# ArseneAmoya/image-retrieval-wavelet

Hardware: AMD Instinct MI355X
Metric: query images/sec + mAP@5000, MIRFLICKR-25k 64-bit hash, 1/2/4/8 MI355X (higher is better)
Workload: dtype f32; 1 GPU; c1: MIRFLICKR-25k shape, retrieval-only: per GPU per step 2048 query images 3x224x224 u8 -> SWT db2 L3 -> band-attention head (Nq=4, E=384; DINOv2 backbone out of scope, CLS features synthetic) -> 64-bit hash -> Hamming top-5000 vs 25,000 codes -> mAP@5000; queries_per_gpu=2048, db_codes=25000, nbits=64, k=5000, wavelet=db2, level=3, arithmetic=fp32 SWT and head (fp32 MFMA), 64-bit popcount ranking, AP in fp32/fp64, streams=1, clock_steps=40, backend=none, parallelism=single GPU

## Files before the change

### image-retrieval-wavelet_amd/csrc/common.hpp

```cpp
#pragma once
#include <hip/hip_runtime.h>
#include <hip/hip_bf16.h>
#include <algorithm>
#include <cstdlib>
#include <cstdio>
#include <cstring>
#include <stdint.h>
#include <stdio.h>
#include <stdarg.h>

#include "twin.hpp"

namespace wv {

const char *tune(const char *name);

#define WV_CHECK_LAUNCH(what)                                                        \
    do {                                                                             \
        hipError_t e_ = hipGetLastError();                                           \
        if (e_ != hipSuccess) WV_FAIL(WV_EHIP, "%s: %s", what, hipGetErrorString(e_)); \
    } while (0)

static inline int64_t ceil_div(int64_t a, int64_t b) { return (a + b - 1) / b; }
static inline int64_t align_up(int64_t a, int64_t b) { return ceil_div(a, b) * b; }

size_t dist_prepared_bytes(int64_t N, int words);
int dist_prepare(const uint64_t *db, void *dbP, int64_t N, int words, hipStream_t st);

constexpr int kWave = 64;
constexpr int kMaxLdsBytes = 160 * 1024;

__device__ __forceinline__ int lane_id() { return threadIdx.x & 63; }
__device__ __forceinline__ int wave_id() { return threadIdx.x >> 6; }

__device__ __forceinline__ uint32_t own_byte(int v)
{
    asm volatile("" : "+v"(v));
    return (uint32_t)v;
}

__device__ __forceinline__ int mbcnt(uint64_t mask)
{
    return __builtin_amdgcn_mbcnt_hi((uint32_t)(mask >> 32),
                                     __builtin_amdgcn_mbcnt_lo((uint32_t)mask, 0));
}

__device__ __forceinline__ uint32_t wave_incl_scan_u32(uint32_t v)
{
    v += (uint32_t)__builtin_amdgcn_update_dpp(0, (int)v, 0x111, 0xf, 0xf, false);
    v += (uint32_t)__builtin_amdgcn_update_dpp(0, (int)v, 0x112, 0xf, 0xf, false);
    v += (uint32_t)__builtin_amdgcn_update_dpp(0, (int)v, 0x114, 0xf, 0xf, false);
    v += (uint32_t)__builtin_amdgcn_update_dpp(0, (int)v, 0x118, 0xf, 0xf, false);
    v += (uint32_t)__builtin_amdgcn_update_dpp(0, (int)v, 0x142, 0xa, 0xf, false);
    v += (uint32_t)__builtin_amdgcn_update_dpp(0, (int)v, 0x143, 0xc, 0xf, false);
    return v;
}

__device__ __forceinline__ uint32_t wave_sum_u32(uint32_t v)
{
    return (uint32_t)__builtin_amdgcn_readlane((int)wave_incl_scan_u32(v), 63);
}

__device__ __forceinline__ double wave_sum_f64(double v)
{
#pragma unroll
    for (int d = 32; d > 0; d >>= 1) v += __shfl_xor(v, d, 64);
    return v;
}

__device__ __forceinline__ float gelu_erf(float v)
{
#ifdef WV_HF_EXACT_ERF
    return 0.5f * v * (1.0f + erff(v * 0.70710678118654752440f));
#else
    const float x = fabsf(v) * 0.70710678118654752440f;
    const float t = __builtin_amdgcn_rcpf(fmaf(0.3275911f, x, 1.0f));
    float p = fmaf(1.061405429f, t, -1.453152027f);
    p = fmaf(p, t, 1.421413741f);
    p = fmaf(p, t, -0.284496736f);
    p = fmaf(p, t, 0.254829592f);
    const float erfc_abs = p * t * __expf(-x * x);
    return 0.5f * v * (v >= 0.f ? 2.0f - erfc_abs : erfc_abs);
#endif
}

}
```

### image-retrieval-wavelet_amd/csrc/head.hip

```cpp
#include "head.hpp"

namespace wv {

template <int TM, int TN, int EPI>
__global__ __launch_bounds__(256) void k_gemm_nt(const float *__restrict__ A, const float *__restrict__ W,
                                                 const float *__restrict__ bias,
                                                 const float *__restrict__ R, int rmod,
                                                 float *__restrict__ C, int M, int N, int K)
{
    const int lane = lane_id(), wv = wave_id();
    const int r = lane & 31, h = lane >> 5;
    const int64_t i0 = (int64_t)blockIdx.y * (64 * TM) + (wv >> 1) * (32 * TM);
    const int64_t j0 = (int64_t)blockIdx.x * (64 * TN) + (wv & 1) * (32 * TN);
    if (i0 >= M || j0 >= N) return;
    f32x16 acc[TM][TN];
#pragma unroll
    for (int a = 0; a < TM; ++a)
#pragma unroll
        for (int b = 0; b < TN; ++b)
#pragma unroll
            for (int e = 0; e < 16; ++e) acc[a][b][e] = 0.f;
    const float *arow[TM], *brow[TN];
#pragma unroll
    for (int a = 0; a < TM; ++a) arow[a] = A + min(i0 + a * 32 + r, (int64_t)M - 1) * K;
// ... 143 lines not shown
            const int lin = blockIdx.y * gridDim.x + blockIdx.x;
            const int tile = (lin % 8) * (total / 8) + lin / 8;
            by = tile / gridDim.x;
            bx = tile - by * gridDim.x;
        }
    }
    const int64_t m0 = (int64_t)by * BM, n0 = (int64_t)bx * BN;

    f32x16 acc[3];
#pragma unroll
    for (int b = 0; b < 3; ++b)
#pragma unroll
        for (int e = 0; e < 16; ++e) acc[b][e] = 0.f;

    f32x4 ra[A4], rb[B4];
    const float *ga[A4], *gb[B4];
    int so_a[A4], so_b[B4];
#pragma unroll
    for (int i = 0; i < A4; ++i) {
        const int ch = i * 256 + tid, row = ch / CPR, c4 = ch % CPR;
        ga[i] = A + min(m0 + row, (int64_t)M - 1) * K + 4 * c4;
        so_a[i] = row * LDP + 4 * c4;
    }
#pragma unroll
    for (int i = 0; i < B4; ++i) {
        const int ch = i * 256 + tid, row = ch / CPR, c4 = ch % CPR;
        gb[i] = W + min(n0 + row, (int64_t)N - 1) * K + 4 * c4;
        so_b[i] = BM * LDP + row * LDP + 4 * c4;
    }
    constexpr int STAGE = (BM + BN) * LDP;
#pragma unroll
    for (int i = 0; i < A4; ++i) ra[i] = *reinterpret_cast<const f32x4 *>(ga[i]);
#pragma unroll
    for (int i = 0; i < B4; ++i) rb[i] = *reinterpret_cast<const f32x4 *>(gb[i]);
#pragma unroll
    for (int i = 0; i < A4; ++i) *reinterpret_cast<f32x4 *>(sm + so_a[i]) = ra[i];
#pragma unroll
    for (int i = 0; i < B4; ++i) *reinterpret_cast<f32x4 *>(sm + so_b[i]) = rb[i];
    const int nk = kchunk / BK;
    if (nk > 1) {
#pragma unroll
        for (int i = 0; i < A4; ++i) ra[i] = *reinterpret_cast<const f32x4 *>(ga[i] + BK);
#pragma unroll
        for (int i = 0; i < B4; ++i) rb[i] = *reinterpret_cast<const f32x4 *>(gb[i] + BK);
    }
    __syncthreads();
    for (int kt = 0; kt < nk; ++kt) {
        float *cur = sm + (kt & 1) * STAGE;
        float *nxt = sm + ((kt & 1) ^ 1) * STAGE;
        if (kt + 1 < nk) {
#pragma unroll
            for (int i = 0; i < A4; ++i) *reinterpret_cast<f32x4 *>(nxt + so_a[i]) = ra[i];
#pragma unroll
            for (int i = 0; i < B4; ++i) *reinterpret_cast<f32x4 *>(nxt + so_b[i]) = rb[i];
        }
        if (kt + 2 < nk) {
            const int k0 = (kt + 2) * BK;
#pragma unroll
            for (int i = 0; i < A4; ++i) ra[i] = *reinterpret_cast<const f32x4 *>(ga[i] + k0);
#pragma unroll
            for (int i = 0; i < B4; ++i) rb[i] = *reinterpret_cast<const f32x4 *>(gb[i] + k0);
        }
        const float *as = cur + (wv * 32 + r) * LDP + 4 * h;
        const float *bs = cur + BM * LDP + r * LDP + 4 * h;
        f32x4 av_n = *reinterpret_cast<const f32x4 *>(as), bv_n[3];
#pragma unroll
        for (int b = 0; b < 3; ++b) bv_n[b] = *reinterpret_cast<const f32x4 *>(bs + b * 32 * LDP);
#pragma unroll
        for (int c = 0; c < BK / 8; ++c) {
            const f32x4 av = av_n;
            f32x4 bv[3];
#pragma unroll
            for (int b = 0; b < 3; ++b) bv[b] = bv_n[b];
            if (c + 1 < BK / 8) {
                av_n = *reinterpret_cast<const f32x4 *>(as + 8 * (c + 1));
#pragma unroll
                for (int b = 0; b < 3; ++b) bv_n[b] = *reinterpret_cast<const f32x4 *>(bs + b * 32 * LDP + 8 * (c + 1));
            }
            __builtin_amdgcn_sched_barrier(0);
#pragma unroll
            for (int b = 0; b < 3; ++b) acc[b] = __builtin_amdgcn_mfma_f32_32x32x2f32(av.x, bv[b].x, acc[b], 0, 0, 0);
#pragma unroll
            for (int b = 0; b < 3; ++b) acc[b] = __builtin_amdgcn_mfma_f32_32x32x2f32(av.y, bv[b].y, acc[b], 0, 0, 0);
#pragma unroll
            for (int b = 0; b < 3; ++b) acc[b] = __builtin_amdgcn_mfma_f32_32x32x2f32(av.z, bv[b].z, acc[b], 0, 0, 0);
#pragma unroll
            for (int b = 0; b < 3; ++b) acc[b] = __builtin_amdgcn_mfma_f32_32x32x2f32(av.w, bv[b].w, acc[b], 0, 0, 0);
        }
        __syncthreads();
    }
    const int64_t row0 = m0 + wv * 32 + 4 * h, col0 = n0 + r;
    if (m0 + BM <= M && n0 + BN <= N) {
#pragma unroll
        for (int b = 0; b < 3; ++b) store_block<EPI, false, true>(acc[b], row0, col0 + b * 32, bias, R, rmod, C, M, N);
    } else {
#pragma unroll
        for (int b = 0; b < 3; ++b) store_block<EPI, true, true>(acc[b], row0, col0 + b * 32, bias, R, rmod, C, M, N);
    }
}

__global__ __launch_bounds__(256) void k_attn_core(const float *__restrict__ Qp,
                                                   const float *__restrict__ KV,
                                                   float *__restrict__ ctx, int B, int E, int heads,
                                                   int Nq, int S)
{
    extern __shared__ float4 sm4[];
    float *kv = reinterpret_cast<float *>(sm4);
    const int KP = 2 * E + 4;
    float *q = kv + (size_t)S * KP;
    float *P = q + (size_t)Nq * E;
    const int b = blockIdx.x, tid = threadIdx.x;
    const int hd = E / heads;
    const float scale = 1.0f / sqrtf((float)hd);
    const int row4 = 2 * E / 4;
    for (int t = tid; t < S * row4; t += blockDim.x) {
        const int s = t / row4, c = t - s * row4;
        *reinterpret_cast<float4 *>(kv + (size_t)s * KP + 4 * c) =
            *reinterpret_cast<const float4 *>(KV + ((size_t)s * B + b) * 2 * E + 4 * c);
    }
    for (int t = tid; t < Nq * E / 4; t += blockDim.x)
        *reinterpret_cast<float4 *>(q + 4 * t) = *reinterpret_cast<const float4 *>(Qp + 4 * t);
    __syncthreads();
    const int ndots = Nq * heads * S;
    for (int t = tid; t < ndots; t += blockDim.x) {
        const int s = t % S, hh = (t / S) % heads, i = t / (S * heads);
        const float *qv = q + (size_t)i * E + hh * hd;
        const float *kr = kv + (size_t)s * KP + hh * hd;
        float acc = 0.f;
        for (int d = 0; d < hd; ++d) acc = fmaf(qv[d], kr[d], acc);
        P[t] = acc * scale;
    }
    __syncthreads();
    for (int t = tid; t < Nq * heads; t += blockDim.x) {
        float *p = P + (size_t)t * S;
        float mx = p[0];
        for (int s = 1; s < S; ++s) mx = fmaxf(mx, p[s]);
        float sum = 0.f;
        for (int s = 0; s < S; ++s) {
            p[s] = expf(p[s] - mx);
            sum += p[s];
        }
        for (int s = 0; s < S; ++s) p[s] = p[s] / sum;
    }
    __syncthreads();
    for (int t = tid; t < Nq * E; t += blockDim.x) {
        const int e = t % E, i = t / E, hh = e / hd;
        const float *p = P + ((size_t)i * heads + hh) * S;
        float acc = 0.f;
        for (int s = 0; s < S; ++s) acc = fmaf(p[s], kv[(size_t)s * KP + E + e], acc);
        ctx[((size_t)b * Nq + i) * E + e] = acc;
    }
}

template <int NV>
__global__ __launch_bounds__(256) void k_layernorm(const float *__restrict__ x, const float *__restrict__ w,
                                                   const float *__restrict__ bvec, float *__restrict__ y,
                                                   int64_t rows, int E, float eps, int nparts)
{
    const int lane = lane_id();
    const int64_t row = (int64_t)blockIdx.x * 4 + wave_id();
    if (row >= rows) return;
    const float *xr = x + row * E;
    const size_t pstride = (size_t)rows * E;
    auto value = [&](int e) {
        float a = xr[e];
        for (int q = 1; q < nparts; ++q) a += xr[q * pstride + e];
        return a;
    };
    float val[NV > 0 ? NV : 1];
    float s = 0.f;
    if constexpr (NV > 0) {
#pragma unroll
        for (int j = 0; j < NV; ++j) {
            const int e = lane + 64 * j;
            val[j] = e < E ? value(e) : 0.f;
            s += val[j];
        }
    } else {
        for (int e = lane; e < E; e += 64) s += value(e);
    }
#pragma unroll
    for (int d = 32; d > 0; d >>= 1) s += __shfl_xor(s, d, 64);
    const float mean = s / (float)E;
    float v = 0.f;
    if constexpr (NV > 0) {
#pragma unroll
        for (int j = 0; j < NV; ++j) {
            const float dlt = lane + 64 * j < E ? val[j] - mean : 0.f;
            v = fmaf(dlt, dlt, v);
        }
    } else {
        for (int e = lane; e < E; e += 64) {
            const float dlt = value(e) - mean;
            v = fmaf(dlt, dlt, v);
        }
    }
#pragma unroll
    for (int d = 32; d > 0; d >>= 1) v += __shfl_xor(v, d, 64);
    const float rstd = 1.0f / sqrtf(v / (float)E + eps);
    if constexpr (NV > 0) {
#pragma unroll
        for (int j = 0; j < NV; ++j) {
            const int e = lane + 64 * j;
            if (e < E) y[row * E + e] = (val[j] - mean) * rstd * w[e] + bvec[e];
        }
    } else {
        for (int e = lane; e < E; e += 64) y[row * E + e] = (value(e) - mean) * rstd * w[e] + bvec[e];
    }
}

void launch_layernorm(const float *x, const float *w, const float *b, float *y, int64_t rows, int E, float eps, int nparts,
                      hipStream_t st)
{
    const dim3 grid((unsigned)ceil_div(rows, 4));
    if (E <= 512) hipLaunchKernelGGL(k_layernorm<8>, grid, dim3(256), 0, st, x, w, b, y, rows, E, eps, nparts);
    else if (E <= 1024) hipLaunchKernelGGL(k_layernorm<16>, grid, dim3(256), 0, st, x, w, b, y, rows, E, eps, nparts);
    else hipLaunchKernelGGL(k_layernorm<0>, grid, dim3(256), 0, st, x, w, b, y, rows, E, eps, nparts);
}

__global__ __launch_bounds__(256) void k_qproj(const float *__restrict__ q, const float *__restrict__ W,
                                               const float *__restrict__ b, float *__restrict__ Qp, int Nq, int E)
{
    const int lane = lane_id(), o = blockIdx.x * 4 + wave_id();
    if (o >= Nq * E) return;
    const int n = o / E, e = o - n * E;
    const float *wr = W + (size_t)e * E, *qr = q + (size_t)n * E;
    float a = 0.f;
    for (int k = lane; k < E; k += 64) a = fmaf(qr[k], wr[k], a);
#pragma unroll
    for (int d = 32; d > 0; d >>= 1) a += __shfl_xor(a, d, 64);
    if (lane == 0) Qp[o] = a + b[e];
}

__global__ void k_mean_rows(const float *__restrict__ x, float *__restrict__ y, int64_t groups, int n, int E)
{
    const int64_t total = groups * E;
    for (int64_t i = (int64_t)blockIdx.x * blockDim.x + threadIdx.x; i < total;
         i += (int64_t)gridDim.x * blockDim.x) {
        const int64_t g = i / E;
        const int e = (int)(i - g * E);
        float s = 0.f;
        for (int j = 0; j < n; ++j) s += x[(g * n + j) * E + e];
        y[i] = s / (float)n;
    }
}

__global__ __launch_bounds__(256) void k_hash_tail(const float *__restrict__ fused, int B, int E,
                                                   const float *__restrict__ hw, const float *__restrict__ hb,
                                                   const float *__restrict__ bn_w, const float *__restrict__ bn_b,
                                                   const float *__restrict__ bn_mean,
                                                   const float *__restrict__ bn_var, float eps, int nbits,
                                                   float *__restrict__ logits_out,
                                                   float *__restrict__ codes_out,
                                                   uint64_t *__restrict__ packed_out)
{
    extern __shared__ float xrow[];
    const int b = blockIdx.x, tid = threadIdx.x, lane = lane_id();
    for (int e = tid; e < E; e += blockDim.x) xrow[e] = fused[(size_t)b * E + e];
    __syncthreads();
    const int words = (nbits + 63) / 64;
    for (int j0 = 0; j0 < words * 64; j0 += blockDim.x) {
        const int j = j0 + tid;
        float v = 0.f;
        const bool valid = j < nbits;
        if (valid) {
            const float4 *wr = reinterpret_cast<const float4 *>(hw + (size_t)j * E);
            float acc = 0.f;
            for (int e4 = 0; e4 < E / 4; ++e4) {
                const float4 w4 = wr[e4];
                acc = fmaf(w4.x, xrow[4 * e4 + 0], acc);
                acc = fmaf(w4.y, xrow[4 * e4 + 1], acc);
                acc = fmaf(w4.z, xrow[4 * e4 + 2], acc);
                acc = fmaf(w4.w, xrow[4 * e4 + 3], acc);
            }
            v = acc + (hb ? hb[j] : 0.f);
            if (bn_w) v = (v - bn_mean[j]) / sqrtf(bn_var[j] + eps) * bn_w[j] + bn_b[j];
            if (logits_out) logits_out[(size_t)b * nbits + j] = v;
            if (codes_out) codes_out[(size_t)b * nbits + j] = v > 0.f ? 1.f : (v < 0.f ? -1.f : (v == 0.f ? 0.f : v));
        }
        const uint64_t word = __ballot(valid && v > 0.f);
        if (packed_out && lane == 0 && j < words * 64) packed_out[(size_t)b * words + j / 64] = word;
    }
}

__global__ __launch_bounds__(256) void k_hash_tail16(const float *__restrict__ fused, int B, int E,
                                                     const float *__restrict__ hw, const float *__restrict__ hb,
                                                     const float *__restrict__ bn_w, const float *__restrict__ bn_b,
                                                     const float *__restrict__ bn_mean,
                                                     const float *__restrict__ bn_var, float eps, int nbits,
                                                     float *__restrict__ logits_out,
                                                     float *__restrict__ codes_out,
                                                     uint64_t *__restrict__ packed_out)
{
    extern __shared__ float4 hsm4[];
    float4 *xs4 = hsm4;
    float *Wt = reinterpret_cast<float *>(hsm4 + 4 * E);
    const int tid = threadIdx.x, lane = lane_id(), wv = wave_id();
    const int b0 = blockIdx.x * 16;
    {
        float *xs = reinterpret_cast<float *>(xs4);
#pragma unroll 8
        for (int i = tid; i < 16 * E; i += 256) {
            const int sidx = i / E, e = i - sidx * E, b = b0 + sidx;
            xs[((sidx >> 2) * E + e) * 4 + (sidx & 3)] = b < B ? fused[(size_t)b * E + e] : 0.f;
        }
    }
    const int words = (nbits + 63) / 64, E4 = E / 4;
    for (int wd = 0; wd < words; ++wd) {
        __syncthreads();
        constexpr int UN = 8;
        for (int base = 0; base < 64 * E4; base += 256 * UN) {
            f32x4 w4[UN];
#pragma unroll
            for (int u = 0; u < UN; ++u) {
                const int i = base + u * 256 + tid, jj = i / E4, e4 = i - jj * E4, j = wd * 64 + jj;
                w4[u] = f32x4{0.f, 0.f, 0.f, 0.f};
                if (i < 64 * E4 && j < nbits) w4[u] = *reinterpret_cast<const f32x4 *>(hw + (size_t)j * E + 4 * e4);
            }
#pragma unroll
            for (int u = 0; u < UN; ++u) {
                const int i = base + u * 256 + tid, jj = i / E4, e4 = i - jj * E4;
                if (i < 64 * E4) {
                    Wt[(4 * e4 + 0) * 65 + jj] = w4[u].x;
                    Wt[(4 * e4 + 1) * 65 + jj] = w4[u].y;
                    Wt[(4 * e4 + 2) * 65 + jj] = w4[u].z;
                    Wt[(4 * e4 + 3) * 65 + jj] = w4[u].w;
                }
            }
        }
        __syncthreads();
        const int j = wd * 64 + lane;
        const bool valid = j < nbits;
        float a0 = 0.f, a1 = 0.f, a2 = 0.f, a3 = 0.f;
        const float4 *xw = xs4 + wv * E;
#pragma unroll 16
        for (int e = 0; e < E; ++e) {
            const float w = Wt[e * 65 + lane];
            const float4 x = xw[e];
            a0 = fmaf(w, x.x, a0);
            a1 = fmaf(w, x.y, a1);
            a2 = fmaf(w, x.z, a2);
            a3 = fmaf(w, x.w, a3);
        }
        float scale = 1.f, shift = 0.f, mean = 0.f, bias = 0.f;
        if (valid) {
            bias = hb ? hb[j] : 0.f;
            if (bn_w) { mean = bn_mean[j]; scale = sqrtf(bn_var[j] + eps); shift = bn_b[j]; }
        }
        const float acc[4] = {a0, a1, a2, a3};
#pragma unroll
        for (int u = 0; u < 4; ++u) {
            const int b = b0 + 4 * wv + u;
            float v = acc[u] + bias;
            if (bn_w && valid) v = (v - mean) / scale * bn_w[j] + shift;
            const bool on = valid && b < B;
            if (on) {
                if (logits_out) logits_out[(size_t)b * nbits + j] = v;
                if (codes_out) codes_out[(size_t)b * nbits + j] = v > 0.f ? 1.f : (v < 0.f ? -1.f : (v == 0.f ? 0.f : v));
            }
            const uint64_t word = __ballot(on && v > 0.f);
            if (packed_out && lane == 0 && b < B) packed_out[(size_t)b * words + wd] = word;
        }
    }
}

__global__ __launch_bounds__(256) void k_hash_tail_mfma(const float *__restrict__ fused, int B, int E,
                                                        const float *__restrict__ hw, const float *__restrict__ hb,
                                                        const float *__restrict__ bn_w, const float *__restrict__ bn_b,
                                                        const float *__restrict__ bn_mean,
                                                        const float *__restrict__ bn_var, float eps, int nbits,
                                                        float *__restrict__ logits_out, float *__restrict__ codes_out,
                                                        uint64_t *__restrict__ packed_out)
{
    __shared__ float part[4][16][64];
    const int lane = lane_id(), wv = wave_id(), r = lane & 31, h = lane >> 5;
    const int b0 = blockIdx.x * 32, n = blockIdx.y;
    const int cpw = E / 32;
    const float *arow = fused + (size_t)min(b0 + r, B - 1) * E + (size_t)wv * cpw * 8 + 4 * h;
    const float *brow = hw + (size_t)min(n * 32 + r, nbits - 1) * E + (size_t)wv * cpw * 8 + 4 * h;
    f32x16 acc[2];
#pragma unroll
    for (int i = 0; i < 2; ++i)
#pragma unroll
        for (int e = 0; e < 16; ++e) acc[i][e] = 0.f;
    constexpr int CB = 12;
    for (int c0 = 0; c0 < cpw; c0 += CB) {
        f32x4 av[CB], bv[CB];
#pragma unroll
        for (int u = 0; u < CB; ++u) {
            const int c = min(c0 + u, cpw - 1);
            av[u] = *reinterpret_cast<const f32x4 *>(arow + 8 * c);
            bv[u] = *reinterpret_cast<const f32x4 *>(brow + 8 * c);
        }
#pragma unroll
        for (int u = 0; u < CB; ++u) {
            if (c0 + u < cpw) {
                acc[u & 1] = __builtin_amdgcn_mfma_f32_32x32x2f32(av[u].x, bv[u].x, acc[u & 1], 0, 0, 0);
                acc[u & 1] = __builtin_amdgcn_mfma_f32_32x32x2f32(av[u].y, bv[u].y, acc[u & 1], 0, 0, 0);
                acc[u & 1] = __builtin_amdgcn_mfma_f32_32x32x2f32(av[u].z, bv[u].z, acc[u & 1], 0, 0, 0);
                acc[u & 1] = __builtin_amdgcn_mfma_f32_32x32x2f32(av[u].w, bv[u].w, acc[u & 1], 0, 0, 0);
            }
        }
    }
#pragma unroll
    for (int e = 0; e < 16; ++e) part[wv][e][lane] = acc[0][e] + acc[1][e];
    __syncthreads();
    const int words = (nbits + 63) / 64;
    const int j = 32 * n + r;
    const bool valid = j < nbits;
    float bias = 0.f, mean = 0.f, scale = 1.f, gain = 1.f, shift = 0.f;
    if (valid) {
        bias = hb ? hb[j] : 0.f;
        if (bn_w) { mean = bn_mean[j]; scale = sqrtf(bn_var[j] + eps); gain = bn_w[j]; shift = bn_b[j]; }
    }
#pragma unroll
    for (int ee = 0; ee < 4; ++ee) {
        const int e = 4 * wv + ee;
        const int b = b0 + 8 * (e >> 2) + 4 * h + (e & 3);
        float v = ((part[0][e][lane] + part[1][e][lane]) + part[2][e][lane]) + part[3][e][lane];
        v += bias;
        if (bn_w) v = (v - mean) / scale * gain + shift;
        if (valid && b < B) {
            if (logits_out) logits_out[(size_t)b * nbits + j] = v;
            if (codes_out) codes_out[(size_t)b * nbits + j] = v > 0.f ? 1.f : (v < 0.f ? -1.f : (v == 0.f ? 0.f : v));
        }
        const uint64_t bal = __ballot(valid && v > 0.f);
        if (packed_out && r == 0 && b < B)
            reinterpret_cast<uint32_t *>(packed_out)[((size_t)b * words + (n >> 1)) * 2 + (n & 1)] = (uint32_t)(bal >> (32 * h));
    }
    if (packed_out && n == (int)gridDim.y - 1 && (gridDim.y & 1) && wv == 0 && lane < 32 && b0 + lane < B)
        reinterpret_cast<uint32_t *>(packed_out)[((size_t)(b0 + lane) * words + (n >> 1)) * 2 + 1] = 0u;
}

template <int TM, int TN, int EPI>
static void launch_gemm_nt(const float *A, const float *W, const float *bias, const float *R, int rmod, float *C,
                           int M, int N, int K, hipStream_t st)
{
    dim3 grid((unsigned)ceil_div(N, 64 * TN), (unsigned)ceil_div(M, 64 * TM));
    hipLaunchKernelGGL((k_gemm_nt<TM, TN, EPI>), grid, dim3(256), 0, st, A, W, bias, R, rmod, C, M, N, K);
}

template <int BM, int BN, int EPI>
static void launch_gemm_lds(const float *A, const float *W, const float *bias, const float *R, int rmod, float *C,
                            int M, int N, int K, hipStream_t st)
{
    constexpr size_t lds = (size_t)2 * (BM + BN) * 36 * sizeof(float);
    auto kern = k_gemm_lds<BM, BN, EPI>;
    if (lds > 64 * 1024)
        (void)hipFuncSetAttribute(reinterpret_cast<const void *>(kern), hipFuncAttributeMaxDynamicSharedMemorySize, (int)lds);
    dim3 grid((unsigned)ceil_div(N, BN), (unsigned)ceil_div(M, BM));
    hipLaunchKernelGGL(kern, grid, dim3(256), lds, st, A, W, bias, R, rmod, C, M, N, K);
}

template <int BK, int EPI>
static void launch_gemm_panel(const float *A, const float *W, const float *bias, const float *R, int rmod, float *C,
                              int M, int N, int K, int ksplit, hipStream_t st)
{
    constexpr size_t lds = (size_t)2 * (128 + 96) * (BK + 4) * sizeof(float);
    auto kern = k_gemm_panel<BK, EPI>;
    if (lds > 64 * 1024)
        (void)hipFuncSetAttribute(reinterpret_cast<const void *>(kern), hipFuncAttributeMaxDynamicSharedMemorySize, (int)lds);
    dim3 grid((unsigned)ceil_div(N, 96), (unsigned)ceil_div(M, 128), (unsigned)ksplit);
    hipLaunchKernelGGL(kern, grid, dim3(256), lds, st, A, W, bias, R, rmod, C, M, N, K, K / ksplit);
}

struct PathF32 {
    using Hidden = float;
    template <int EPI>
    static void gemm(GemmPlan g, const float *A, const float *W, const float *bias, const float *R, int rmod, float *C, int M,
                     int N, int K, hipStream_t st)
    {
        switch (g.kernel) {
        case Gemm::nt64: return launch_gemm_nt<1, 1, EPI>(A, W, bias, R, rmod, C, M, N, K, st);
        case Gemm::nt128: return launch_gemm_nt<2, 2, EPI>(A, W, bias, R, rmod, C, M, N, K, st);
        case Gemm::lds64: return launch_gemm_lds<64, 64, EPI>(A, W, bias, R, rmod, C, M, N, K, st);
        case Gemm::lds128x64: return launch_gemm_lds<128, 64, EPI>(A, W, bias, R, rmod, C, M, N, K, st);
        case Gemm::lds128: return launch_gemm_lds<128, 128, EPI>(A, W, bias, R, rmod, C, M, N, K, st);
        case Gemm::panel32: return launch_gemm_panel<32, EPI>(A, W, bias, R, rmod, C, M, N, K, g.ksplit, st);
        case Gemm::panel64: return launch_gemm_panel<64, EPI>(A, W, bias, R, rmod, C, M, N, K, g.ksplit, st);
        default: return;
        }
    }
};

void launch_gemm_f32(GemmPlan g, const float *A, const float *W, const float *bias, float *C, int M, int N, int K, hipStream_t st)
{
    PathF32::gemm<EPI_NONE>(g, A, W, bias, nullptr, 1, C, M, N, K, st);
}

void launch_qproj(const wv_head_params *p, float *Qp, hipStream_t st)
{
    hipLaunchKernelGGL(k_qproj, dim3((unsigned)ceil_div(p->num_queries * p->embed_dim, 4)), dim3(256), 0, st, p->q_eff,
                       p->in_proj_w, p->in_proj_b, Qp, p->num_queries, p->embed_dim);
}

void launch_attn_core(const wv_head_params *p, const HeadPlan &pl, const float *Qp, const float *KV, float *ctx, int B, hipStream_t st)
{
    if (pl.attn_lds > 64 * 1024)
        (void)hipFuncSetAttribute(reinterpret_cast<const void *>(k_attn_core), hipFuncAttributeMaxDynamicSharedMemorySize,
                                  (int)pl.attn_lds);
    hipLaunchKernelGGL(k_attn_core, dim3(B), dim3(256), pl.attn_lds, st, Qp, KV, ctx, B, p->embed_dim, p->num_heads,
                       p->num_queries, p->num_tokens);
}

void launch_mean_rows(const float *x, float *y, int64_t groups, int n, int E, hipStream_t st)
{
    hipLaunchKernelGGL(k_mean_rows, dim3((unsigned)std::min<int64_t>(ceil_div(groups * E, 256), 4096)), dim3(256), 0, st, x, y,
                       groups, n, E);
}

}

using namespace wv;

extern "C" size_t wv_band_attn_pool_workspace_bytes(const wv_head_params *p, int B)
{
    return head_plan(p, B, HeadPrec::f32).ws.bytes;
}

extern "C" int wv_band_attn_qproj(const wv_head_params *p, float *q_proj_out, void *stream)
{
    HeadPlan pl{};
    if (!head_check_params(p, 1, pl)) WV_FAIL(pl.rc, "%s", pl.why);
    WV_REQUIRE(q_proj_out, "band_attn_qproj: null buffer");
    launch_qproj(p, q_proj_out, (hipStream_t)stream);
    WV_CHECK_LAUNCH("k_qproj");
    return WV_OK;
}

extern "C" size_t wv_band_attn_prepared_bytes(const wv_head_params *p)
{
    if (!p) return 0;
    const HeadPlan pl = head_plan(p, 1, HeadPrec::f32);
    if (pl.rc) {
        set_error("%s", pl.why);
        return 0;
    }
    return head_front_prepared_bytes(p);
}

extern "C" int wv_band_attn_prepare(const wv_head_params *p, void *prepared_out, void *stream)
{
    HeadPlan pl{};
    if (!head_check_params(p, 1, pl)) WV_FAIL(pl.rc, "%s", pl.why);
    WV_REQUIRE(prepared_out, "band_attn_prepare: null buffer");
    if (!head_front_has_kernel(p))
        WV_FAIL(WV_ENOTSUP, "band_attn_prepare: no fused kernel for E=%d S=%d Nq=%d heads=%d", p->embed_dim, p->num_tokens,
                p->num_queries, p->num_heads);
    return head_front_prepare(p, prepared_out, (hipStream_t)stream);
}

extern "C" int wv_band_attn_pool(const wv_head_params *p, const float *feats, int B, float *out,
                                 void *workspace, size_t workspace_bytes, void *stream)
{
    const HeadPlan pl = head_plan(p, B, HeadPrec::f32);
    if (pl.rc) WV_FAIL(pl.rc, "%s", pl.why);
    WV_REQUIRE(feats && out, "band_attn_pool: null buffer");
    WV_REQUIRE((int64_t)B * std::max(p->num_queries, p->num_tokens) < (1ll << 31), "band_attn_pool: B=%d too large", B);
    if (B == 0) return WV_OK;
    if (!workspace || workspace_bytes < pl.ws.bytes)
        WV_FAIL(WV_ENOMEM, "band_attn_pool: workspace %zu < %zu bytes", workspace_bytes, pl.ws.bytes);
    hipStream_t st = (hipStream_t)stream;
    const float *Qp = p->q_proj ? p->q_proj : reinterpret_cast<const float *>(p->prepared);
    if (!Qp && !pl.front) {
        launch_qproj(p, ws_at<float>(workspace, pl.ws.Qp), st);
        Qp = ws_at<float>(workspace, pl.ws.Qp);
    }
    const size_t E = p->embed_dim;
    const HeadWeights<float> w{p->in_proj_w + E * E, p->attn_out_w, p->mlp0_w, p->mlp2_w, p->out_w};
    head_run_stages<PathF32>(p, pl, w, Qp, feats, B, out, workspace, st);
    WV_CHECK_LAUNCH("band_attn_pool");
    return WV_OK;
}

extern "C" int wv_hash_tail(const float *fused, int B, int E, const float *hash_w, const float *hash_b,
                            const float *bn_w, const float *bn_b, const float *bn_mean,
                            const float *bn_var, float bn_eps, int nbits, float *logits_out,
                            float *codes_out, uint64_t *packed_out, void *stream)
{
    WV_REQUIRE(fused && hash_w, "hash_tail: null buffer");
    WV_REQUIRE(B >= 0 && E >= 4 && E % 4 == 0 && nbits >= 1, "hash_tail: bad shape B=%d E=%d nbits=%d", B, E, nbits);
    WV_REQUIRE(!bn_w || (bn_b && bn_mean && bn_var), "hash_tail: incomplete BatchNorm parameters");
    WV_REQUIRE(E * sizeof(float) <= 48 * 1024, "hash_tail: E=%d too large", E);
    if (B == 0) return WV_OK;
    const size_t lds16 = ((size_t)4 * E * 4 + (size_t)E * 65) * sizeof(float);
    const char *pin = ::wv::tune("WV_HASH_TAIL");
    const bool simple = pin && !strcmp(pin, "simple");
    if (!simple && !(pin && !strcmp(pin, "valu16")) && E % 32 == 0 && (B >= 32 || (pin && !strcmp(pin, "mfma")))) {
        const dim3 grid((unsigned)ceil_div(B, 32), (unsigned)ceil_div(nbits, 32));
        hipLaunchKernelGGL(k_hash_tail_mfma, grid, dim3(256), 0, (hipStream_t)stream, fused, B, E, hash_w, hash_b, bn_w, bn_b,
                           bn_mean, bn_var, bn_eps, nbits, logits_out, codes_out, packed_out);
    } else if (lds16 <= (size_t)kMaxLdsBytes - 1024 && B >= 64 && !simple) {
        if (lds16 > 64 * 1024)
            (void)hipFuncSetAttribute(reinterpret_cast<const void *>(k_hash_tail16), hipFuncAttributeMaxDynamicSharedMemorySize, (int)lds16);
        hipLaunchKernelGGL(k_hash_tail16, dim3((unsigned)ceil_div(B, 16)), dim3(256), lds16, (hipStream_t)stream, fused, B,
                           E, hash_w, hash_b, bn_w, bn_b, bn_mean, bn_var, bn_eps, nbits, logits_out, codes_out,
                           packed_out);
    } else {
        hipLaunchKernelGGL(k_hash_tail, dim3(B), dim3(256), E * sizeof(float), (hipStream_t)stream, fused, B, E,
                           hash_w, hash_b, bn_w, bn_b, bn_mean, bn_var, bn_eps, nbits, logits_out, codes_out,
                           packed_out);
    }
    WV_CHECK_LAUNCH("k_hash_tail");
    return WV_OK;
}
```

### image-retrieval-wavelet_amd/csrc/head_front.hip

```cpp
#include "head.hpp"

namespace wv {

constexpr int HF_E = 384;
constexpr int HF_LDA = HF_E + 4;
constexpr int HF_KC = HF_E / 8;
constexpr int HF_D = 4;
constexpr int HF_ENTRY4 = 3 * 64;
constexpr int HF_TILE = 32 * HF_LDA;

struct HeadFrontPlan {
    int ok, nq, heads, nsc, kw, ns;
    int nsp;
    size_t entries;
    size_t wave_stride4;
    size_t qp_bytes, bytes;
};

static HeadFrontPlan head_front_plan(const wv_head_params *p)
{
    HeadFrontPlan g{};
    if (!p || p->embed_dim != HF_E || p->num_tokens != 4 || (p->num_queries != 4 && p->num_queries != 8)) return g;
    if (p->num_heads < 1 || HF_E % p->num_heads) return g;
    const int cols = p->num_queries * p->num_heads;
// ... 46 lines not shown
                a[1] = fmaf(qv[d], kv.y, a[1]);
                a[2] = fmaf(qv[d], kv.z, a[2]);
                a[3] = fmaf(qv[d], kv.w, a[3]);
            }
            v = f32x4{a[0] * scale, a[1] * scale, a[2] * scale, a[3] * scale};
        }
    } else if (entry >= (size_t)nsp && entry < entries) {
        size_t m = entry - nsp;
        const int n = 96 * w + 32 * slot + r;
        const float *src;
        if (m < (size_t)HF_KC) src = in_proj_w + (size_t)2 * E * E + (size_t)n * E + 8 * m + 4 * h;
        else if (m < (size_t)2 * HF_KC) src = Wo + (size_t)n * E + 8 * (m - HF_KC) + 4 * h;
        else {
            m -= 2 * HF_KC;
            const int j = (int)(m / (2 * HF_KC)), mm = (int)(m % (2 * HF_KC));
            if (mm < HF_KC) src = W0 + (size_t)(E * j + n) * E + 8 * mm + 4 * h;
            else src = W2 + (size_t)n * (4 * E) + E * j + 8 * (mm - HF_KC) + 4 * h;
        }
        v = *reinterpret_cast<const f32x4 *>(src);
    }
    stream[idx] = v;
}

#ifdef WV_HF_STAMPS
__device__ unsigned long long g_hf_stamps[16];
#define HF_STAMP(i) do { __builtin_amdgcn_sched_barrier(0); const unsigned long long now_ = __builtin_amdgcn_s_memtime(); \
    asm volatile("s_waitcnt lgkmcnt(0)" ::: "memory"); if (threadIdx.x == 0) atomicAdd(&g_hf_stamps[i], now_ - stamp_); stamp_ = now_; \
    __builtin_amdgcn_sched_barrier(0); } while (0)
#define HF_STAMP_INIT unsigned long long stamp_ = __builtin_amdgcn_s_memtime()
#else
#define HF_STAMP(i) do { } while (0)
#define HF_STAMP_INIT do { } while (0)
#endif

__device__ __forceinline__ void lds_barrier() { asm volatile("s_waitcnt lgkmcnt(0)\n\ts_barrier" ::: "memory"); }

#define HF_MFMA(a, b, c) __builtin_amdgcn_mfma_f32_32x32x2f32((a), (b), (c), 0, 0, 0)


template <int NE>
__device__ __forceinline__ void gemm_stream(f32x16 (&acc)[3], f32x4 (&ring)[HF_D][3], const f32x4 *&wq, const float *arow)
{
    static_assert(NE % HF_D == 0, "phase length must be a multiple of the ring depth");
    f32x4 av_n = *reinterpret_cast<const f32x4 *>(arow);
    for (int c = 0; c < NE; c += HF_D) {
#pragma unroll
        for (int d = 0; d < HF_D; ++d) {
            constexpr int D = HF_D;
            const int slot = (d + D - 1) % D;
            const f32x4 av = av_n;
            const int cn = min(c + d + 1, NE - 1);
            ring[slot][0] = wq[(size_t)(d * 3 + 0) * 64];
            av_n = *reinterpret_cast<const f32x4 *>(arow + 8 * cn);
            __builtin_amdgcn_sched_barrier(0);
#pragma unroll
            for (int b = 0; b < 3; ++b) acc[b] = HF_MFMA(av.x, ring[d][b].x, acc[b]);
            __builtin_amdgcn_sched_barrier(0);
            ring[slot][1] = wq[(size_t)(d * 3 + 1) * 64];
            __builtin_amdgcn_sched_barrier(0);
#pragma unroll
            for (int b = 0; b < 3; ++b) acc[b] = HF_MFMA(av.y, ring[d][b].y, acc[b]);
            __builtin_amdgcn_sched_barrier(0);
            ring[slot][2] = wq[(size_t)(d * 3 + 2) * 64];
            __builtin_amdgcn_sched_barrier(0);
#pragma unroll
            for (int b = 0; b < 3; ++b) acc[b] = HF_MFMA(av.z, ring[d][b].z, acc[b]);
#pragma unroll
            for (int b = 0; b < 3; ++b) acc[b] = HF_MFMA(av.w, ring[d][b].w, acc[b]);
            __builtin_amdgcn_sched_barrier(0);
        }
        wq += (size_t)HF_D * HF_ENTRY4;
    }
}

template <int NE, int NREAL>
__device__ __forceinline__ void scores_stream(f32x16 (&sacc)[3], f32x4 (&ring)[HF_D][3], const f32x4 *&wq, const float *arow)
{
    static_assert(NE % HF_D == 0, "phase length must be a multiple of the ring depth");
    f32x4 a_n[3];
#pragma unroll
    for (int t = 0; t < 3; ++t) a_n[t] = *reinterpret_cast<const f32x4 *>(arow + 8 * t);
    for (int c = 0; c < NE; c += HF_D) {
#pragma unroll
        for (int d = 0; d < HF_D; ++d) {
            constexpr int D = HF_D;
            const int slot = (d + D - 1) % D;
#pragma unroll
            for (int b = 0; b < 3; ++b) ring[slot][b] = wq[(size_t)(d * 3 + b) * 64];
            f32x4 a[3];
#pragma unroll
            for (int t = 0; t < 3; ++t) a[t] = a_n[t];
            const int cn = min(c + d + 1, NREAL - 1);
#pragma unroll
            for (int t = 0; t < 3; ++t) a_n[t] = *reinterpret_cast<const f32x4 *>(arow + 8 * (3 * cn + t));
            __builtin_amdgcn_sched_barrier(0);
#pragma unroll
            for (int t = 0; t < 3; ++t) sacc[t] = HF_MFMA(a[t].x, ring[d][t].x, sacc[t]);
#pragma unroll
            for (int t = 0; t < 3; ++t) sacc[t] = HF_MFMA(a[t].y, ring[d][t].y, sacc[t]);
#pragma unroll
            for (int t = 0; t < 3; ++t) sacc[t] = HF_MFMA(a[t].z, ring[d][t].z, sacc[t]);
#pragma unroll
            for (int t = 0; t < 3; ++t) sacc[t] = HF_MFMA(a[t].w, ring[d][t].w, sacc[t]);
            __builtin_amdgcn_sched_barrier(0);
        }
        wq += (size_t)HF_D * HF_ENTRY4;
    }
}

__device__ __forceinline__ void zero_acc(f32x16 (&acc)[3])
{
#pragma unroll
    for (int b = 0; b < 3; ++b)
#pragma unroll
        for (int e = 0; e < 16; ++e) acc[b][e] = 0.f;
}

__device__ __forceinline__ float half_reduce16(const float (&v)[16], int r)
{
    float a[8], b[4], c[2];
    const bool u4 = r & 16, u3 = r & 8, u2 = r & 4, u1 = r & 2;
#pragma unroll
    for (int k = 0; k < 8; ++k) a[k] = (u4 ? v[k + 8] : v[k]) + __shfl_xor(u4 ? v[k] : v[k + 8], 16, 64);
#pragma unroll
    for (int k = 0; k < 4; ++k) b[k] = (u3 ? a[k + 4] : a[k]) + __shfl_xor(u3 ? a[k] : a[k + 4], 8, 64);
#pragma unroll
    for (int k = 0; k < 2; ++k) c[k] = (u2 ? b[k + 2] : b[k]) + __shfl_xor(u2 ? b[k] : b[k + 2], 4, 64);
    float d = (u1 ? c[1] : c[0]) + __shfl_xor(u1 ? c[0] : c[1], 2, 64);
    d += __shfl_xor(d, 1, 64);
    return d;
}

template <int NQ, int NSC>
__global__ __launch_bounds__(256, 1) void k_head_front(const float *__restrict__ feats, const f32x4 *__restrict__ stream,
                                                       size_t wave_stride4, const float *__restrict__ bv,
                                                       const float *__restrict__ bo, const float *__restrict__ q_eff,
                                                       const float *__restrict__ ln_w, const float *__restrict__ ln_b,
                                                       const float *__restrict__ b0, const float *__restrict__ b2,
                                                       float *__restrict__ x2, int B, int heads, float eps)
{
    constexpr int E = HF_E, LDA = HF_LDA, SPB = 32 / NQ, KW = 4 / NSC, NS = (HF_KC / KW) / 3;
    constexpr int SPP = 33;
    extern __shared__ float4 hf_sm4[];
    float *T0 = reinterpret_cast<float *>(hf_sm4);
    float *H = T0 + HF_TILE;
    float *SP = H;
    float *P = H + 4 * 32 * SPP;
    float *ST = H + HF_TILE;
    const int tid = threadIdx.x, lane = lane_id(), wv = wave_id(), r = lane & 31, h = lane >> 5;
    const int hd = E / heads;
    const int s0 = blockIdx.x * SPB;

    HF_STAMP_INIT;
    f32x4 ring[HF_D][3];
    const f32x4 *wq = stream + (size_t)wv * wave_stride4 + lane;
#pragma unroll
    for (int d = 0; d < HF_D - 1; ++d)
#pragma unroll
        for (int b = 0; b < 3; ++b) ring[d][b] = wq[(size_t)(d * 3 + b) * 64];
    wq += (size_t)(HF_D - 1) * HF_ENTRY4;
    float c_bv[3], c_bo[3], c_lw[3], c_lb[3], c_b2[3], c_b0[4][3], c_q[NQ][3];
#pragma unroll
    for (int b = 0; b < 3; ++b) {
        const int col = 96 * wv + 32 * b + r;
        c_bv[b] = bv[col];
        c_bo[b] = bo[col];
        c_lw[b] = ln_w[col];
        c_lb[b] = ln_b[col];
        c_b2[b] = b2[col];
#pragma unroll
        for (int j = 0; j < 4; ++j) c_b0[j][b] = b0[E * j + col];
#pragma unroll
        for (int i = 0; i < NQ; ++i) c_q[i][b] = q_eff[i * E + col];
    }

    for (int i = tid; i < 32 * (E / 4); i += 256) {
        const int rr = i / (E / 4), c4 = i - rr * (E / 4), bl = rr >> 2, s = rr & 3;
        f32x4 v = {0.f, 0.f, 0.f, 0.f};
        if (bl < SPB && s0 + bl < B) v = *reinterpret_cast<const f32x4 *>(feats + ((size_t)s * B + s0 + bl) * E + 4 * c4);
        *reinterpret_cast<f32x4 *>(T0 + rr * LDA + 4 * c4) = v;
    }
    lds_barrier();
    HF_STAMP(0);
    const float *arow0 = T0 + r * LDA + 4 * h;
    f32x16 acc[3];

    {
        zero_acc(acc);
        const int kpart = wv % KW;
        scores_stream<(NS + HF_D - 1) / HF_D * HF_D, NS>(acc, ring, wq, arow0 + 8 * kpart * (HF_KC / KW));
#pragma unroll
        for (int e = 0; e < 16; ++e) {
            const int row = 8 * (e >> 2) + 4 * h + (e & 3);
            SP[(wv * 32 + row) * SPP + r] = (acc[0][e] + acc[1][e]) + acc[2][e];
        }
    }
    lds_barrier();
    HF_STAMP(1);
    for (int it = tid; it < SPB * NQ * heads; it += 256) {
        const int hh = it % heads, bi = it / heads, bl = bi / NQ, i = bi - bl * NQ;
        const int sc = i * heads + hh, sb = sc >> 5, col = sc & 31;
        float p[4];
#pragma unroll
        for (int s = 0; s < 4; ++s) {
            float a = SP[((sb * KW) * 32 + 4 * bl + s) * SPP + col];
#pragma unroll
            for (int k = 1; k < KW; ++k) a += SP[((sb * KW + k) * 32 + 4 * bl + s) * SPP + col];
            p[s] = a;
        }
        const float mx = fmaxf(fmaxf(p[0], p[1]), fmaxf(p[2], p[3]));
        float sum = 0.f;
#pragma unroll
        for (int s = 0; s < 4; ++s) {
            p[s] = expf(p[s] - mx);
            sum += p[s];
        }
        *reinterpret_cast<f32x4 *>(P + (size_t)it * 4) = f32x4{p[0] / sum, p[1] / sum, p[2] / sum, p[3] / sum};
    }

    HF_STAMP(2);
    zero_acc(acc);
    gemm_stream<HF_KC>(acc, ring, wq, arow0);
    lds_barrier();
    HF_STAMP(3);
#pragma unroll
    for (int b = 0; b < 3; ++b) {
        const int col = 96 * wv + 32 * b + r, hh = col / hd;
        const float bias = c_bv[b];
#pragma unroll
        for (int j = 0; j < 4; ++j) {
            const int bl = h + 2 * j;
            if (bl < SPB) {
                const float v0 = acc[b][4 * j] + bias, v1 = acc[b][4 * j + 1] + bias, v2 = acc[b][4 * j + 2] + bias,
                            v3 = acc[b][4 * j + 3] + bias;
#pragma unroll
                for (int i = 0; i < NQ; ++i) {
                    const f32x4 p4 = *reinterpret_cast<const f32x4 *>(P + ((size_t)(bl * NQ + i) * heads + hh) * 4);
                    float c = p4.x * v0;
                    c = fmaf(p4.y, v1, c);
                    c = fmaf(p4.z, v2, c);
                    c = fmaf(p4.w, v3, c);
                    T0[(bl * NQ + i) * LDA + col] = c;
                }
            }
        }
    }
    lds_barrier();
    HF_STAMP(4);

    zero_acc(acc);
    gemm_stream<HF_KC>(acc, ring, wq, arow0);
    HF_STAMP(5);
    {
        float rs[16];
#pragma unroll
        for (int e = 0; e < 16; ++e) rs[e] = 0.f;
#pragma unroll
        for (int b = 0; b < 3; ++b)
#pragma unroll
            for (int e = 0; e < 16; ++e) {
                const float qv = NQ == 4 ? c_q[e & 3][b] : (h ? c_q[(4 + (e & 3)) % NQ][b] : c_q[e & 3][b]);
                acc[b][e] = acc[b][e] + c_bo[b] + qv;
                rs[e] += acc[b][e];
            }
        const int erow = r >> 1, srow = 8 * (erow >> 2) + 4 * h + (erow & 3);
        {
            const float t = half_reduce16(rs, r);
            if (!(r & 1)) ST[wv * 32 + srow] = t;
        }
        lds_barrier();
        float mean[16];
#pragma unroll
        for (int e = 0; e < 16; ++e) {
            const int row = 8 * (e >> 2) + 4 * h + (e & 3);
            mean[e] = (((ST[row] + ST[32 + row]) + ST[64 + row]) + ST[96 + row]) * (1.0f / (float)E);
            rs[e] = 0.f;
        }
#pragma unroll
        for (int b = 0; b < 3; ++b)
#pragma unroll
            for (int e = 0; e < 16; ++e) {
                acc[b][e] -= mean[e];
                rs[e] = fmaf(acc[b][e], acc[b][e], rs[e]);
            }
        {
            const float t = half_reduce16(rs, r);
            if (!(r & 1)) ST[128 + wv * 32 + srow] = t;
        }
        lds_barrier();
#pragma unroll
        for (int e = 0; e < 16; ++e) {
            const int row = 8 * (e >> 2) + 4 * h + (e & 3);
            const float var = (((ST[128 + row] + ST[160 + row]) + ST[192 + row]) + ST[224 + row]) * (1.0f / (float)E);
            mean[e] = 1.0f / sqrtf(var + eps);
        }
#pragma unroll
        for (int b = 0; b < 3; ++b) {
            const int col = 96 * wv + 32 * b + r;
#pragma unroll
            for (int e = 0; e < 16; ++e) {
                const int row = 8 * (e >> 2) + 4 * h + (e & 3);
                T0[row * LDA + col] = acc[b][e] * mean[e] * c_lw[b] + c_lb[b];
            }
        }
    }
    lds_barrier();
    HF_STAMP(6);

    f32x16 xacc[3];
    zero_acc(xacc);
#pragma unroll 1
    for (int j = 0; j < 4; ++j) {
        zero_acc(acc);
        gemm_stream<HF_KC>(acc, ring, wq, arow0);
        HF_STAMP(7);
        float *Hj = H + (j & 1) * HF_TILE;
#pragma unroll
        for (int b = 0; b < 3; ++b) {
            const int col = 96 * wv + 32 * b + r;
            const float bias = j == 0 ? c_b0[0][b] : j == 1 ? c_b0[1][b] : j == 2 ? c_b0[2][b] : c_b0[3][b];
#pragma unroll
            for (int e = 0; e < 16; ++e) {
                const int row = 8 * (e >> 2) + 4 * h + (e & 3);
                Hj[row * LDA + col] = gelu_erf(acc[b][e] + bias);
            }
        }
        lds_barrier();
        HF_STAMP(8);
        gemm_stream<HF_KC>(xacc, ring, wq, Hj + r * LDA + 4 * h);
        HF_STAMP(9);
    }
#pragma unroll
    for (int b = 0; b < 3; ++b) {
        const int col = 96 * wv + 32 * b + r;
#pragma unroll
        for (int e = 0; e < 16; ++e) {
            const int row = 8 * (e >> 2) + 4 * h + (e & 3);
            const int64_t grow = (int64_t)blockIdx.x * 32 + row;
            if (grow < (int64_t)B * NQ) x2[grow * E + col] = xacc[b][e] + c_b2[b] + T0[row * LDA + col];
        }
    }
    HF_STAMP(10);
}

int head_front_prepare(const wv_head_params *p, void *prepared, hipStream_t st)
{
    const HeadFrontPlan g = head_front_plan(p);
    float *Qp = reinterpret_cast<float *>(prepared);
    launch_qproj(p, Qp, st);
    WV_CHECK_LAUNCH("k_qproj");
    f32x4 *stream = reinterpret_cast<f32x4 *>(reinterpret_cast<char *>(prepared) + g.qp_bytes);
    const size_t total = 4 * g.wave_stride4;
    hipLaunchKernelGGL(k_head_pack, dim3((unsigned)ceil_div((int64_t)total, 256)), dim3(256), 0, st, p->in_proj_w, Qp,
                       p->attn_out_w, p->mlp0_w, p->mlp2_w, stream, g.nq, g.heads, g.kw, g.ns, g.nsp, g.entries, g.wave_stride4);
    WV_CHECK_LAUNCH("k_head_pack");
    return WV_OK;
}

template <int NQ, int NSC>
static void launch_front(const HeadFrontPlan &g, const wv_head_params *p, const float *feats, int B, float *x2, hipStream_t st)
{
    constexpr size_t lds = (size_t)3 * HF_TILE * sizeof(float);
    static_assert(lds <= (size_t)kMaxLdsBytes, "three tiles must fit the CU's LDS");
    auto kern = k_head_front<NQ, NSC>;
    (void)hipFuncSetAttribute(reinterpret_cast<const void *>(kern), hipFuncAttributeMaxDynamicSharedMemorySize, (int)lds);
    const f32x4 *stream = reinterpret_cast<const f32x4 *>(reinterpret_cast<const char *>(p->prepared) + g.qp_bytes);
    hipLaunchKernelGGL(kern, dim3((unsigned)ceil_div(B, 32 / NQ)), dim3(256), lds, st, feats, stream, g.wave_stride4,
                       p->in_proj_b + 2 * HF_E, p->attn_out_b, p->q_eff, p->norm1_w, p->norm1_b, p->mlp0_b, p->mlp2_b, x2, B,
                       p->num_heads, p->ln_eps);
}

void head_front_launch(const wv_head_params *p, const float *feats, int B, float *x2, hipStream_t st)
{
    const HeadFrontPlan g = head_front_plan(p);
    if (g.nq == 4 && g.nsc == 1) launch_front<4, 1>(g, p, feats, B, x2, st);
    else if (g.nq == 4 && g.nsc == 2) launch_front<4, 2>(g, p, feats, B, x2, st);
    else if (g.nq == 4 && g.nsc == 4) launch_front<4, 4>(g, p, feats, B, x2, st);
    else if (g.nq == 8 && g.nsc == 1) launch_front<8, 1>(g, p, feats, B, x2, st);
    else if (g.nq == 8 && g.nsc == 2) launch_front<8, 2>(g, p, feats, B, x2, st);
    else if (g.nq == 8 && g.nsc == 4) launch_front<8, 4>(g, p, feats, B, x2, st);
}

}

#ifdef WV_HF_STAMPS
extern "C" int wv_debug_hf_stamps(unsigned long long *host16)
{
    if (hipMemcpyFromSymbol(host16, HIP_SYMBOL(wv::g_hf_stamps), 16 * sizeof(unsigned long long)) != hipSuccess) return -5;
    unsigned long long zero[16] = {0};
    if (hipMemcpyToSymbol(HIP_SYMBOL(wv::g_hf_stamps), zero, sizeof(zero)) != hipSuccess) return -5;
    return 0;
}
#endif
```

Measured before the change: 1.600 million query images/s.

## Reorder head-front loads, pack GELU in pairs, template layernorm on slice count

The fused head-front kernel now issues the feature-tile global loads into registers first, then the constant loads and the weight-ring prefetch, and only afterwards writes the tile to LDS, with sched barriers to keep that order. The goal is to overlap global load latency. GELU is evaluated two elements at a time with a packed float2 helper, and the residual reads from LDS are hoisted ahead of the output store loop. Layernorm is templated on the number of k-split partial slices and gets an E<=384 instantiation, so partial-sum loads and gain/bias loads are unrolled and issued up front; unsupported slice counts abort. Debug exports are also added. These changes raise register pressure and could lower occupancy.

```diff
diff --git a/image-retrieval-wavelet_amd/csrc/common.hpp b/image-retrieval-wavelet_amd/csrc/common.hpp
--- a/image-retrieval-wavelet_amd/csrc/common.hpp
+++ b/image-retrieval-wavelet_amd/csrc/common.hpp
@@ -84,4 +84,25 @@
 #endif
 }
 
+using f32x2 = __attribute__((ext_vector_type(2))) float;
+__device__ __forceinline__ f32x2 gelu_erf2(f32x2 v)
+{
+#ifdef WV_HF_EXACT_ERF
+    return f32x2{gelu_erf(v.x), gelu_erf(v.y)};
+#else
+    const f32x2 x = __builtin_elementwise_abs(v) * 0.70710678118654752440f;
+    const f32x2 d = __builtin_elementwise_fma(f32x2{0.3275911f, 0.3275911f}, x, f32x2{1.0f, 1.0f});
+    const f32x2 t = {__builtin_amdgcn_rcpf(d.x), __builtin_amdgcn_rcpf(d.y)};
+    f32x2 p = __builtin_elementwise_fma(f32x2{1.061405429f, 1.061405429f}, t, f32x2{-1.453152027f, -1.453152027f});
+    p = __builtin_elementwise_fma(p, t, f32x2{1.421413741f, 1.421413741f});
+    p = __builtin_elementwise_fma(p, t, f32x2{-0.284496736f, -0.284496736f});
+    p = __builtin_elementwise_fma(p, t, f32x2{0.254829592f, 0.254829592f});
+    const f32x2 a = -x * x;
+    const f32x2 erfc_abs = p * t * f32x2{__expf(a.x), __expf(a.y)};
+    const f32x2 two = f32x2{2.0f, 2.0f} - erfc_abs;
+    const f32x2 s = {v.x >= 0.f ? two.x : erfc_abs.x, v.y >= 0.f ? two.y : erfc_abs.y};
+    return 0.5f * v * s;
+#endif
 }
+
+}
diff --git a/image-retrieval-wavelet_amd/csrc/head.hip b/image-retrieval-wavelet_amd/csrc/head.hip
--- a/image-retrieval-wavelet_amd/csrc/head.hip
+++ b/image-retrieval-wavelet_amd/csrc/head.hip
@@ -319,10 +319,10 @@
     }
 }
 
-template <int NV>
+template <int NV, int NP>
 __global__ __launch_bounds__(256) void k_layernorm(const float *__restrict__ x, const float *__restrict__ w,
                                                    const float *__restrict__ bvec, float *__restrict__ y,
-                                                   int64_t rows, int E, float eps, int nparts)
+                                                   int64_t rows, int E, float eps)
 {
     const int lane = lane_id();
     const int64_t row = (int64_t)blockIdx.x * 4 + wave_id();
@@ -330,17 +330,33 @@
     const float *xr = x + row * E;
     const size_t pstride = (size_t)rows * E;
     auto value = [&](int e) {
-        float a = xr[e];
-        for (int q = 1; q < nparts; ++q) a += xr[q * pstride + e];
+        float part[NP];
+#pragma unroll
+        for (int q = 0; q < NP; ++q) part[q] = xr[q * pstride + e];
+        float a = part[0];
+#pragma unroll
+        for (int q = 1; q < NP; ++q) a += part[q];
         return a;
     };
-    float val[NV > 0 ? NV : 1];
+    float val[NV > 0 ? NV : 1], gain[NV > 0 ? NV : 1], shift[NV > 0 ? NV : 1];
     float s = 0.f;
     if constexpr (NV > 0) {
+        float part[NP][NV];
+#pragma unroll
+        for (int q = 0; q < NP; ++q)
+#pragma unroll
+            for (int j = 0; j < NV; ++j) part[q][j] = xr[q * pstride + min(lane + 64 * j, E - 1)];
 #pragma unroll
         for (int j = 0; j < NV; ++j) {
-            const int e = lane + 64 * j;
-            val[j] = e < E ? value(e) : 0.f;
+            gain[j] = w[min(lane + 64 * j, E - 1)];
+            shift[j] = bvec[min(lane + 64 * j, E - 1)];
+        }
+#pragma unroll
+        for (int j = 0; j < NV; ++j) {
+            float a = part[0][j];
+#pragma unroll
+            for (int q = 1; q < NP; ++q) a += part[q][j];
+            val[j] = lane + 64 * j < E ? a : 0.f;
             s += val[j];
         }
     } else {
@@ -369,20 +385,40 @@
 #pragma unroll
         for (int j = 0; j < NV; ++j) {
             const int e = lane + 64 * j;
-            if (e < E) y[row * E + e] = (val[j] - mean) * rstd * w[e] + bvec[e];
+            if (e < E) y[row * E + e] = (val[j] - mean) * rstd * gain[j] + shift[j];
         }
     } else {
         for (int e = lane; e < E; e += 64) y[row * E + e] = (value(e) - mean) * rstd * w[e] + bvec[e];
     }
 }
 
+using LayerNormKernel = void (*)(const float *, const float *, const float *, float *, int64_t, int, float);
+
+template <int NP> static LayerNormKernel layernorm_rows(int E)
+{
+    return E <= 384 ? k_layernorm<6, NP> : E <= 512 ? k_layernorm<8, NP> : E <= 1024 ? k_layernorm<16, NP> : k_layernorm<0, NP>;
+}
+
+static LayerNormKernel layernorm_kernel(int E, int nparts)
+{
+    switch (nparts) {
+    case 1: return layernorm_rows<1>(E);
+    case 2: return layernorm_rows<2>(E);
+    case 4: return layernorm_rows<4>(E);
+    case 8: return layernorm_rows<8>(E);
+    default: return nullptr;
+    }
+}
+
 void launch_layernorm(const float *x, const float *w, const float *b, float *y, int64_t rows, int E, float eps, int nparts,
                       hipStream_t st)
 {
-    const dim3 grid((unsigned)ceil_div(rows, 4));
-    if (E <= 512) hipLaunchKernelGGL(k_layernorm<8>, grid, dim3(256), 0, st, x, w, b, y, rows, E, eps, nparts);
-    else if (E <= 1024) hipLaunchKernelGGL(k_layernorm<16>, grid, dim3(256), 0, st, x, w, b, y, rows, E, eps, nparts);
-    else hipLaunchKernelGGL(k_layernorm<0>, grid, dim3(256), 0, st, x, w, b, y, rows, E, eps, nparts);
+    const LayerNormKernel kern = layernorm_kernel(E, nparts);
+    if (!kern) {
+        fprintf(stderr, "wvhash: k_layernorm has no instantiation for %d slices\n", nparts);
+        abort();
+    }
+    hipLaunchKernelGGL(kern, dim3((unsigned)ceil_div(rows, 4)), dim3(256), 0, st, x, w, b, y, rows, E, eps);
 }
 
 __global__ __launch_bounds__(256) void k_qproj(const float *__restrict__ q, const float *__restrict__ W,
@@ -680,6 +716,13 @@
 
 using namespace wv;
 
+extern "C" int wv_debug_readout_slices(int bf16, int M, int N, int K)
+{
+    return bf16 ? readout_ksplit_bf16(M, N, K) : readout_ksplit_f32(M, N, K, ::wv::tune("WV_GEMM"));
+}
+
+extern "C" int wv_debug_layernorm_slices(int E, int nparts) { return layernorm_kernel(E, nparts) != nullptr; }
+
 extern "C" size_t wv_band_attn_pool_workspace_bytes(const wv_head_params *p, int B)
 {
     return head_plan(p, B, HeadPrec::f32).ws.bytes;
diff --git a/image-retrieval-wavelet_amd/csrc/head_front.hip b/image-retrieval-wavelet_amd/csrc/head_front.hip
--- a/image-retrieval-wavelet_amd/csrc/head_front.hip
+++ b/image-retrieval-wavelet_amd/csrc/head_front.hip
@@ -222,13 +222,16 @@
     const int s0 = blockIdx.x * SPB;
 
     HF_STAMP_INIT;
-    f32x4 ring[HF_D][3];
-    const f32x4 *wq = stream + (size_t)wv * wave_stride4 + lane;
-#pragma unroll
-    for (int d = 0; d < HF_D - 1; ++d)
-#pragma unroll
-        for (int b = 0; b < 3; ++b) ring[d][b] = wq[(size_t)(d * 3 + b) * 64];
-    wq += (size_t)(HF_D - 1) * HF_ENTRY4;
+    constexpr int FT = 32 * (E / 4) / 256;
+    static_assert(FT * 256 == 32 * (E / 4), "the feature tile is a whole number of 16-byte loads per thread");
+    f32x4 fv[FT];
+#pragma unroll
+    for (int t = 0; t < FT; ++t) {
+        const int i = tid + 256 * t, rr = i / (E / 4), c4 = i - rr * (E / 4), bl = rr >> 2, s = rr & 3;
+        fv[t] = f32x4{0.f, 0.f, 0.f, 0.f};
+        if (bl < SPB && s0 + bl < B) fv[t] = *reinterpret_cast<const f32x4 *>(feats + ((size_t)s * B + s0 + bl) * E + 4 * c4);
+    }
+    __builtin_amdgcn_sched_barrier(0);
     float c_bv[3], c_bo[3], c_lw[3], c_lb[3], c_b2[3], c_b0[4][3], c_q[NQ][3];
 #pragma unroll
     for (int b = 0; b < 3; ++b) {
@@ -244,11 +247,19 @@
         for (int i = 0; i < NQ; ++i) c_q[i][b] = q_eff[i * E + col];
     }
 
-    for (int i = tid; i < 32 * (E / 4); i += 256) {
-        const int rr = i / (E / 4), c4 = i - rr * (E / 4), bl = rr >> 2, s = rr & 3;
-        f32x4 v = {0.f, 0.f, 0.f, 0.f};
-        if (bl < SPB && s0 + bl < B) v = *reinterpret_cast<const f32x4 *>(feats + ((size_t)s * B + s0 + bl) * E + 4 * c4);
-        *reinterpret_cast<f32x4 *>(T0 + rr * LDA + 4 * c4) = v;
+    __builtin_amdgcn_sched_barrier(0);
+    f32x4 ring[HF_D][3];
+    const f32x4 *wq = stream + (size_t)wv * wave_stride4 + lane;
+#pragma unroll
+    for (int d = 0; d < HF_D - 1; ++d)
+#pragma unroll
+        for (int b = 0; b < 3; ++b) ring[d][b] = wq[(size_t)(d * 3 + b) * 64];
+    wq += (size_t)(HF_D - 1) * HF_ENTRY4;
+    __builtin_amdgcn_sched_barrier(0);
+#pragma unroll
+    for (int t = 0; t < FT; ++t) {
+        const int i = tid + 256 * t, rr = i / (E / 4), c4 = i - rr * (E / 4);
+        *reinterpret_cast<f32x4 *>(T0 + rr * LDA + 4 * c4) = fv[t];
     }
     lds_barrier();
     HF_STAMP(0);
@@ -390,9 +401,11 @@
             const int col = 96 * wv + 32 * b + r;
             const float bias = j == 0 ? c_b0[0][b] : j == 1 ? c_b0[1][b] : j == 2 ? c_b0[2][b] : c_b0[3][b];
 #pragma unroll
-            for (int e = 0; e < 16; ++e) {
+            for (int e = 0; e < 16; e += 2) {
                 const int row = 8 * (e >> 2) + 4 * h + (e & 3);
-                Hj[row * LDA + col] = gelu_erf(acc[b][e] + bias);
+                const f32x2 g = gelu_erf2(f32x2{acc[b][e] + bias, acc[b][e + 1] + bias});
+                Hj[row * LDA + col] = g.x;
+                Hj[(row + 1) * LDA + col] = g.y;
             }
         }
         lds_barrier();
@@ -400,6 +413,11 @@
         gemm_stream<HF_KC>(xacc, ring, wq, Hj + r * LDA + 4 * h);
         HF_STAMP(9);
     }
+    float res[3][16];
+#pragma unroll
+    for (int b = 0; b < 3; ++b)
+#pragma unroll
+        for (int e = 0; e < 16; ++e) res[b][e] = T0[(8 * (e >> 2) + 4 * h + (e & 3)) * LDA + 96 * wv + 32 * b + r];
 #pragma unroll
     for (int b = 0; b < 3; ++b) {
         const int col = 96 * wv + 32 * b + r;
@@ -407,7 +425,7 @@
         for (int e = 0; e < 16; ++e) {
             const int row = 8 * (e >> 2) + 4 * h + (e & 3);
             const int64_t grow = (int64_t)blockIdx.x * 32 + row;
-            if (grow < (int64_t)B * NQ) x2[grow * E + col] = xacc[b][e] + c_b2[b] + T0[row * LDA + col];
+            if (grow < (int64_t)B * NQ) x2[grow * E + col] = xacc[b][e] + c_b2[b] + res[b][e];
         }
     }
     HF_STAMP(10);
```

New measurement: 1.612 million query images/s (median of 5 runs). About the same (+0.8%).
